# egor-achkasov/hermespy-rt

Hardware: AMD Instinct MI355X
Metric: resolved propagation paths/sec (higher is better)
Workload: dtype f32; 1 GPU; simple_street_canyon_with_cars.hrt, 1 TX + 4 RX, 4000000 rays/TX, 4 bounces, 3.5 GHz; parallelism=ray-sharded x1 (weak scaling), round-robin 4096-path granules, rays_total=4000000

## Files before the change

hermespy-rt_amd/csrc/host/problem.c:

```c
#include <math.h>
#include <pthread.h>
#include <stdarg.h>
#include <stdio.h>
#include <stdlib.h>
#include <string.h>
#include <time.h>
#include <unistd.h>

#include "hrt_internal.h"
#include "hrt_launch_plan.h"


static __thread char g_err[512];

const char *hrt_last_error(void) { return g_err; }
const char *hrt_version(void) { return "hermespy-rt_amd 0.1 (gfx950)"; }

int hrt_fail(int code, const char *fmt, ...)
{
    va_list ap;
    va_start(ap, fmt);
    vsnprintf(g_err, sizeof g_err, fmt, ap);
    va_end(ap);
    return code;
// ... 1267 lines not shown
{
    HRT_HIP(hrt_hip_set_device(device), "hipSetDevice");
    HRT_HIP(hrt_hip_free(ptr), "hipFree");
    return HRT_OK;
}
int hrt_device_upload(int device, void *dst, const void *src, uint64_t bytes)
{
    HRT_HIP(hrt_hip_set_device(device), "hipSetDevice");
    HRT_HIP(hrt_hip_h2d(dst, src, bytes), "hipMemcpy H2D");
    return HRT_OK;
}
int hrt_device_download(int device, void *dst, const void *src, uint64_t bytes)
{
    HRT_HIP(hrt_hip_set_device(device), "hipSetDevice");
    HRT_HIP(hrt_hip_d2h(dst, src, bytes), "hipMemcpy D2H");
    return HRT_OK;
}
int hrt_device_sync(int device, void *stream)
{
    HRT_HIP(hrt_hip_set_device(device), "hipSetDevice");
    HRT_HIP(hrt_hip_stream_sync(stream), "hipStreamSynchronize");
    return HRT_OK;
}
int hrt_device_mem_info(int device, uint64_t *free_bytes, uint64_t *total_bytes)
{
    HRT_HIP(hrt_hip_set_device(device), "hipSetDevice");
    HRT_HIP(hrt_hip_mem_info(free_bytes, total_bytes), "hipMemGetInfo");
    return HRT_OK;
}


int hrt_selftest_math(int device, int fn, const float *in, float *out, uint64_t n)
{
    if (!in || !out || fn < 0 || fn > 10) return hrt_fail(HRT_E_INVALID, "hrt_selftest_math: bad argument");
    void *d_in = NULL, *d_out = NULL;
    int rc = hrt_device_malloc(device, &d_in, n * 4);
    if (rc) return rc;
    if ((rc = hrt_device_malloc(device, &d_out, n * 4))) { hrt_device_free(device, d_in); return rc; }
    if (!(rc = hrt_device_upload(device, d_in, in, n * 4))) {
        int e = hrt_hip_selftest_math(fn, (const float *)d_in, (float *)d_out, n, NULL);
        if (e) rc = hrt_fail_hip(e, "hrt_selftest_math");
        else if (!(rc = hrt_device_sync(device, NULL))) rc = hrt_device_download(device, out, d_out, n * 4);
    }
    hrt_device_free(device, d_in);
    hrt_device_free(device, d_out);
    return rc;
}


static const void *cand_table(const hrt_problem *p, int mode)
{
    switch (mode) {
    case 0: return p->kpatch.mask;
    case 1: return p->kpatch.num_img ? p->kpatch.mask : NULL;
    case 2: return p->kpatch.txcell;
    case 3: return p->krxt.cell_mask;
    default: return NULL;
    }
}

int hrt_debug_candidates(const hrt_problem *p, int mode, uint64_t n, const float *in, uint32_t *out)
{
    if (!p || !in || !out || mode < 0 || mode > 3) return hrt_fail(HRT_E_INVALID, "hrt_debug_candidates: bad argument");
    if (n > (1ull << 26)) return hrt_fail(HRT_E_INVALID, "hrt_debug_candidates: more than 2^26 queries");
    if (!cand_table(p, mode)) return hrt_fail(HRT_E_INVALID, "hrt_debug_candidates: the problem has no table for mode %d", mode);
    if (n == 0) return HRT_OK;
    void *d_in = NULL, *d_out = NULL;
    int rc = hrt_device_malloc(p->device, &d_in, n * 32);
    if (rc) return rc;
    if ((rc = hrt_device_malloc(p->device, &d_out, n * 40))) { hrt_device_free(p->device, d_in); return rc; }
    if (!(rc = hrt_device_upload(p->device, d_in, in, n * 32))) {
        int e = hrt_hip_debug_candidates(p->d_tri, p->num_tri, p->d_tx_pos, p->num_rx, p->num_tx, &p->kpatch, &p->krxt, mode, n,
                                         (const float *)d_in, (uint32_t *)d_out, NULL);
// ... 41 lines not shown
```

hermespy-rt_amd/csrc/hrt_fused_body.inc:

```
    constexpr int AUX = CHAIN ? 16 : 0;
    const uint32_t tid = threadIdx.x, lane = tid & 63u, wave = tid >> 6;
    uint32_t *counts = reinterpret_cast<uint32_t *>(P.ws + P.off_counts);
    if (!CHAIN && FIRST && blockIdx.x >= gridDim.x - P.los_blocks) {
        los_pairs(P, blockIdx.x - (gridDim.x - P.los_blocks));
        return;
    }
    const uint32_t n_in = CHAIN ? n_in_c : (FIRST ? P.n0 : counts[b]);
    if (!CHAIN && !FIRST && (counts[P.num_bounces + 1] & kErrVoid)) return;
    const uint32_t n_grid = gridDim.x - (FIRST ? P.los_blocks : 0u);
    const uint32_t Ke = CHAIN ? Ke_c : ((K > 1 && n_in <= kShortList && (uint64_t)n_grid * HRT_BLOCK >= n_in) ? 1u : (uint32_t)K);
    const uint32_t MC = Ke * HRT_BLOCK;
    const uint32_t n_chunks = CHAIN ? n_chunks_c : (n_in + MC - 1u) / MC;
    const uint32_t chunk = CHAIN ? chunk_c : blockIdx.x;
    if (!CHAIN && chunk >= n_chunks) return;
    const bool do_trace = FIRST || (b < P.num_bounces);

    const uint32_t T = P.num_tri;
    const uint32_t cap4 = (uint32_t)P.cap * 4u;
    const float4 *g_tri = reinterpret_cast<const float4 *>(P.tri);
    const float2 *g_tg = reinterpret_cast<const float2 *>(P.acc.tg);
    const float4 *g_leaf = reinterpret_cast<const float4 *>(P.acc.leaf);
    const uint32_t n_leaf = P.acc.num_leaf;
    const FusedLds L = fused_lds<TRI_IN_LDS, (VARIANT == 9), FIRST>(lds, T, n_leaf, P.num_rx, wave);
#ifdef HRT_PHASE_STATS
// ... 142 lines not shown

    if constexpr (!FIRST) if (!P.records_done) {
        const uint32_t pb = b - 1;
#pragma unroll
        for (int k = 0; k < K; ++k) {
            const uint32_t i = chunk * MC + (uint32_t)k * HRT_BLOCK + tid;
            const uint32_t i4 = i * 4u;
            if (HRT_BALLOT(valid[k]) == 0ull) continue;
            const Ball ball = (VARIANT >= 2 && VARIANT != 6 && !masked) ? origin_ball(o[k], valid[k])
                                                                       : Ball{{0.f, 0.f, 0.f}, 0.f, false};
            F3 n = {0.f, 0.f, 1.f}, mvel = {0.f, 0.f, 0.f};
            float mat_s = 0.f, mat_alpha = 1.f, th = theta[k];
            if (valid[k]) {
                uint32_t ht = htri[k];
                if (ht >= T) {
                    atomicOr(&counts[P.num_bounces + 1], 4u);
                    ht = 0u;
                }
                const float4 q2 = tri[HRT_ROW * ht + 2];
                n = {q2.y, q2.z, q2.w};
                const uint32_t mesh = __float_as_uint(tri[HRT_ROW * ht + 4].w);
                const float4 mm = gather4(mesh_r, HRT_MESH_FLOATS * 4u, mesh, 0u);
                mvel = {mm.x, mm.y, mm.z};
                const float4 m3 = L.mat[4u * __float_as_uint(mm.w) + 3u];
                mat_s = m3.x;
                mat_alpha = m3.y;
            }
            for (uint32_t rx = 0; rx < P.num_rx; ++rx) {
                const float4 rp = L.rx[rx];
                const F3 apex = {rp.x, rp.y, rp.z};
                float d2rx;
                F3 w = shadow_dir(o[k], apex, d2rx);
                if (!valid[k]) w = {0.f, 0.f, 1.f};
                const Hit sh = masked ? closest_hit_masked(tri, P.acc.orig, P.rxt, rx, T, o[k], w, valid[k], lane, 2)
                                      : closest_hit<VARIANT>(tri, tg, leaf, P.acc, P.rxt, rx, P.acc.orig, T, o[k], w, valid[k],
                                                             lane, ball, true, apex, L.mask, L.wleaf, 2);
                bool unblocked = false;
                if (valid[k]) {
                    const Rsrc rec = rec_blk(P, pb, rx);
                    if (sh.tri != HRT_NO_HIT) {
                        const float4 s2 = tri[HRT_ROW * sh.tri + 2];
                        th = incidence_angle({s2.y, s2.z, s2.w}, w);
                    }
                    if (sh.tri != HRT_NO_HIT && sh.t <= 1.f) {
                        stf(rec, R_A0 * cap4, i4, 0.f);
                        stf(rec, R_A1 * cap4, i4, 0.f);
                        stf(rec, R_A2 * cap4, i4, 0.f);
                        stf(rec, R_A3 * cap4, i4, 0.f);
                        stf(rec, R_TAU * cap4, i4, 0.f);
                    } else {
                        unblocked = true;
                        const float th_s = acos_f_ool(dot3(w, n));
                        const float4 S = scatter_pattern(mat_s, mat_alpha, th_s, th, lds_addr(L.mat + kMatItems));
                        float o0 = a0[k] * S.x - a1[k] * S.y;
                        float o1 = a0[k] * S.y + a1[k] * S.x;
                        float o2 = a2[k] * S.z - a3[k] * S.w;
                        float o3 = a2[k] * S.w + a3[k] * S.z;
                        float f2 = P.fsl_mult * d2rx;
                        f2 *= f2;
                        if (f2 > 1.f) { o0 /= f2; o1 /= f2; o2 /= f2; o3 /= f2; }
                        stf(rec, R_A0 * cap4, i4, o0);
                        stf(rec, R_A1 * cap4, i4, o1);
                        stf(rec, R_A2 * cap4, i4, o2);
                        stf(rec, R_A3 * cap4, i4, o3);
                        stf(rec, R_TAU * cap4, i4, tau[k] + div_c(d2rx));
                        stf(rec, R_DX * cap4, i4, -w.x);
                        stf(rec, R_DY * cap4, i4, -w.y);
// ... 71 lines not shown
```

hermespy-rt_amd/csrc/hrt_kernels.hip:

```cpp
#include <hip/hip_runtime.h>
#include <string.h>

#include <stdint.h>
#include <stdio.h>
#include <stdlib.h>

#include "hrt_kparams.h"
#include "hrt_launch_dir.h"
#include "hrt_launch_plan.h"
#include "hrt_libm.h"

#pragma clang fp contract(off)

namespace {

constexpr float kEps = 1.1920928955078125e-07f;
constexpr float kOnePlusEps = 1.00000011920928955078125f;
constexpr float kPi = 3.14159265358979323846f;
constexpr float kC = 299792458.0f;
constexpr float kInvC = 1.0f / kC;
__device__ __forceinline__ float div_c(float a)
{
    const float q = a * kInvC;
    const float r = __builtin_fmaf(-q, kC, a);
// ... 21 lines not shown
template <typename TriPtr>
__device__ __forceinline__ Hit closest_hit_plain(TriPtr tri, const uint32_t *__restrict__ orig,
                                                 uint32_t num_tri, F3 o, F3 d)
{
    float best = 1e9f;
    uint32_t who = HRT_NO_HIT, who_o = 0u;
    for (uint32_t j = 0; j < num_tri; ++j) {
        const float4 q0 = tri[HRT_ROW * j], q1 = tri[HRT_ROW * j + 1], q2 = tri[HRT_ROW * j + 2];
        const F3 v1 = {q0.x, q0.y, q0.z};
        const F3 e1 = {q0.w, q1.x, q1.y};
        const F3 e2 = {q1.z, q1.w, q2.x};
        const F3 pv = cross3(d, e2);
        const float det = dot3(e1, pv);
        if (det > -kEps && det < kEps) continue;
        const F3 s = sub3(o, v1);
        const float u = dot3(s, pv) / det;
        if (u < -kEps || u > kOnePlusEps) continue;
        const F3 q = cross3(s, e1);
        const float v = dot3(d, q) / det;
        const float w = u + v;
        if (v < -kEps || w > kOnePlusEps) continue;
        const float dist = dot3(e2, q) / det;
        if (dist > kEps && (dist < best || (dist == best && orig[j] < who_o))) {
            best = dist; who = j; who_o = orig[j];
        }
    }
    return {who, best};
}

constexpr float kK1 = 1.1920928955078125e-07f * (1.f + 0x1p-18f);
constexpr float kK2 = 1.f + 0x1p-20f;
constexpr float kK3 = 1.f + 0x1p-19f;
constexpr float kK5 = 1.1920928955078125e-07f * (1.f - 0x1p-18f);

__device__ __forceinline__ uint32_t lane_prefix(unsigned long long mask)
{
    return __builtin_amdgcn_mbcnt_hi((uint32_t)(mask >> 32),
                                     __builtin_amdgcn_mbcnt_lo((uint32_t)mask, 0u));
}

__device__ __forceinline__ bool wave_all(bool p) { return __builtin_amdgcn_ballot_w64(!p) == 0ull; }

__device__ __forceinline__ float xor_sign(float x, uint32_t sign_bit)
{
    return __uint_as_float(__float_as_uint(x) ^ sign_bit);
}

template <typename TriPtr>
__device__ __forceinline__ Hit closest_hit_staged(TriPtr tri, const uint32_t *__restrict__ orig,
                                                  uint32_t num_tri, F3 o, F3 d)
{
    float best = 1e9f;
    uint32_t who = HRT_NO_HIT, who_o = 0u;
    for (uint32_t j = 0; j < num_tri; ++j) {
        const float4 q0 = tri[HRT_ROW * j], q1 = tri[HRT_ROW * j + 1], q2 = tri[HRT_ROW * j + 2];
        const F3 v1 = {q0.x, q0.y, q0.z};
        const F3 e1 = {q0.w, q1.x, q1.y};
        const F3 e2 = {q1.z, q1.w, q2.x};
        const F3 pv = cross3(d, e2);
        const float det = dot3(e1, pv);
        const F3 s = sub3(o, v1);
        const float nu = dot3(s, pv);
        const float a = fabsf(det);
        const uint32_t sg = __float_as_uint(det) & 0x80000000u;
        const float nu_s = xor_sign(nu, sg);
        const float k1a = kK1 * a, k2a = kK2 * a;
// ... 319 lines not shown
#define HRT_STAGED_BODY(J)                                                                      \
    {                                                                                           \
        const float4 q0 = tri[HRT_ROW * (J)], q1 = tri[HRT_ROW * (J) + 1], q2 = tri[HRT_ROW * (J) + 2];           \
        HRT_STAGED_TEST(J, q0, q1, q2)                                                          \
    }
#define HRT_STAGED_TEST(J, q0, q1, q2)                                                          \
    {                                                                                           \
        const F3 v1 = {q0.x, q0.y, q0.z};                                                       \
        const F3 e1 = {q0.w, q1.x, q1.y};                                                       \
        const F3 e2 = {q1.z, q1.w, q2.x};                                                       \
        const F3 pv = cross3(d, e2);                                                            \
        const float det = dot3(e1, pv);                                                         \
        const F3 s = sub3(o, v1);                                                               \
        const float nu = dot3(s, pv);                                                           \
        const float a = fabsf(det);                                                             \
        const uint32_t sg = __float_as_uint(det) & 0x80000000u;                                 \
        const float nu_s = xor_sign(nu, sg);                                                    \
        const float k1a = kK1 * a, k2a = kK2 * a;                                               \
        unsigned long long rm = inval | HRT_BALLOT(a < kEps) | HRT_BALLOT(nu_s < -k1a) |        \
                                HRT_BALLOT(nu_s > k2a);                                         \
        if (rm != ~0ull) {                                                                      \
            HRT_STAT(kind, 3, 1);                                                               \
            const F3 q = cross3(s, e1);                                                         \
            const float nv = dot3(d, q);                                                        \
            const float nv_s = xor_sign(nv, sg);                                                \
            rm |= HRT_BALLOT(nv_s < -k1a) | HRT_BALLOT((nu_s + nv_s) > kK3 * a);                \
            if (rm != ~0ull) {                                                                  \
                HRT_STAT(kind, 4, 1);                                                           \
                const float nt = dot3(e2, q);                                                   \
                const float nt_s = xor_sign(nt, sg);                                            \
                rm |= HRT_BALLOT(nt_s < kK5 * a) | HRT_BALLOT(nt_s > (best * a) * kK2);         \
                if (rm != ~0ull) {                                                              \
                    HRT_STAT(kind, 5, 1);                                                       \
                    const float u = nu / det;                                                   \
                    const float v = nv / det;                                                   \
                    const float w = u + v;                                                      \
                    const float dist = nt / det;                                                \
                    const bool rej = (rm >> lane) & 1ull;                                       \
                    const bool miss = (det > -kEps && det < kEps) | (u < -kEps) |               \
                                      (u > kOnePlusEps) | (v < -kEps) | (w > kOnePlusEps);      \
                    const uint32_t oj = orig[(J)];         \
                    const bool take = !rej & !miss & (dist > kEps) &                            \
                                      ((dist < best) | ((dist == best) & (oj < who_o)));        \
                    best = take ? dist : best;                                                  \
                    who = take ? (J) : who;                                                     \
                    who_o = take ? oj : who_o;                                                  \
                }                                                                               \
            }                                                                                   \
        }                                                                                       \
    }

constexpr uint32_t kMaskRounds = HRT_MASK_ROUNDS;
constexpr uint32_t kCandBuf = HRT_CAND_BUF;
__host__ __device__ constexpr uint32_t wave_scratch4(bool cand_buf) { return HRT_WAVE_SCRATCH4(cand_buf); }

__device__ __forceinline__ uint32_t rxt_cell(F3 a)
{
    const float ax = fabsf(a.x), ay = fabsf(a.y), az = fabsf(a.z);
    uint32_t m = 0u;
    float major = a.x, c1 = a.y, c2 = a.z;
    if (ay > ax && ay >= az) { m = 1u; major = a.y; c1 = a.z; c2 = a.x; }
    else if (az > ax && az > ay) { m = 2u; major = a.z; c1 = a.x; c2 = a.y; }
    const float inv = __builtin_amdgcn_rcpf(major);
    const float u = c1 * inv, v = c2 * inv;
    int iu = (int)((u * 0.5f + 0.5f) * (float)HRT_RXT_N), iv = (int)((v * 0.5f + 0.5f) * (float)HRT_RXT_N);
    iu = iu < 0 ? 0 : (iu > HRT_RXT_N - 1 ? HRT_RXT_N - 1 : iu);
    iv = iv < 0 ? 0 : (iv > HRT_RXT_N - 1 ? HRT_RXT_N - 1 : iv);
    const uint32_t f = m + (major < 0.f ? 3u : 0u);
    return (f * HRT_RXT_N + (uint32_t)iv) * HRT_RXT_N + (uint32_t)iu;
}

__device__ __forceinline__ bool rxt_inside(const hrt_krxt &X, F3 o)
{
    const F3 dc = sub3(o, {X.cx, X.cy, X.cz});
    return fast_sqrt(fdot3(dc, dc)) * 1.0001f <= X.region_r;
}
__device__ __forceinline__ unsigned long long rxt_cell_load(const hrt_krxt &X, uint32_t apex_k, F3 d)
{
    return X.cell_mask[(uint64_t)apex_k * HRT_RXT_BINS + rxt_cell(d)];
}
template <typename TriPtr>
__device__ __forceinline__ Hit closest_hit_masked(TriPtr tri, const uint32_t *__restrict__ orig, const hrt_krxt &X,
                                                  uint32_t apex_k, uint32_t num_tri, F3 o, F3 d, bool valid,
                                                  uint32_t lane, [[maybe_unused]] int kind)
{
    float best = 1e9f;
    uint32_t who = HRT_NO_HIT, who_o = 0u;
    const unsigned long long inval = HRT_BALLOT(!valid);
    if (inval == ~0ull) return {who, best};
    unsigned long long mine = 0ull;
    if (valid) {
        mine = rxt_inside(X, o) ? rxt_cell_load(X, apex_k, d)
                                : (num_tri >= 64u ? ~0ull : ((1ull << num_tri) - 1ull));
    }
    unsigned long long m = wave_or64(mine);
    HRT_STAT(kind, 0, 1);
    HRT_STAT(kind, 1, 1);
    HRT_STAT(kind, 2, __popcll(m));
    while (m) {
        const uint32_t j = (uint32_t)__builtin_ctzll(m);
        m &= m - 1ull;
        HRT_STAGED_BODY(j)
    }
    return {who, best};
}

using Rsrc = __amdgpu_buffer_rsrc_t;
__device__ __forceinline__ Rsrc make_rsrc(const uint8_t *base)
{
    return __builtin_amdgcn_make_buffer_rsrc(const_cast<uint8_t *>(base), 0, 0xffffffff, 0x00020000);
}

__device__ __forceinline__ void wave_or256(uint32_t (&w)[8])
{
    uint32_t c[4];
#pragma unroll
    for (int k = 0; k < 4; ++k) {
        const auto r = __builtin_amdgcn_permlane32_swap(w[k], w[k + 4], false, false);
        c[k] = (uint32_t)r[0] | (uint32_t)r[1];
    }
    uint32_t e[2];
#pragma unroll
    for (int k = 0; k < 2; ++k) {
        const auto r = __builtin_amdgcn_permlane16_swap(c[k], c[k + 2], false, false);
        e[k] = (uint32_t)r[0] | (uint32_t)r[1];
    }
#define HRT_OR2(CTRL) "v_or_b32_dpp %0, %0, %0 " CTRL "\n" "v_or_b32_dpp %1, %1, %1 " CTRL "\n" "s_nop 0\n"
    asm volatile(
        "s_nop 4\n"
        HRT_OR2("row_shr:1 row_mask:0xf bank_mask:0xf")
        HRT_OR2("row_shr:2 row_mask:0xf bank_mask:0xf")
// ... 34 lines not shown
        const float fu = fdot3(sv, {p0.x, p0.y, p0.z}), fv = fdot3(sv, {p1.x, p1.y, p1.z});
        const float hh = fdot3(sv, {q2.y, q2.z, q2.w});
        const uint32_t bits = __float_as_uint(p1.w), nu = bits & 0xffffu, nv = bits >> 16;
        R.served = (nu != 0u) & (fabsf(hh) <= X.hmax) & (fu >= -HRT_PATCH_ACCEPT) & (fv >= -HRT_PATCH_ACCEPT) &
                   (fu <= (float)nu + HRT_PATCH_ACCEPT) & (fv <= (float)nv + HRT_PATCH_ACCEPT);
        if (image) {
            const F3 im = image_of(apex, q0, q2);
            const F3 wv = sub3(o, im);
            const F3 cx = fcross3(wv, d);
            R.served &= (fdot3(cx, cx) <= 0.98f * X.ro_img * X.ro_img) && (fdot3(wv, d) > 0.f);
        }
        const uint32_t iu = min((uint32_t)max((int)floorf(fu), 0), nu - 1u);
        const uint32_t iv = min((uint32_t)max((int)floorf(fv), 0), nv - 1u);
        R.off = (__float_as_uint(p0.w) + iv * nu + iu) * (HRT_PATCH_WORDS * 8u);
    }
    return R;
}

__device__ __forceinline__ void patch_load(const hrt_kpatch &X, const PatchRef R, uint32_t apex_k, bool valid, uint32_t (&w)[8])
{
#pragma unroll
    for (int k = 0; k < 8; ++k) w[k] = 0u;
    if (valid && R.served) {
        const Rsrc mr = make_rsrc(reinterpret_cast<const uint8_t *>(X.mask));
        const uint32_t off = R.off + apex_k * X.num_patch * (HRT_PATCH_WORDS * 8u);
        const auto a = __builtin_amdgcn_raw_buffer_load_b128(mr, (int)off, 0, 0);
        const auto b = __builtin_amdgcn_raw_buffer_load_b128(mr, (int)(off + 16u), 0, 0);
        w[0] = (uint32_t)a[0]; w[1] = (uint32_t)a[1]; w[2] = (uint32_t)a[2]; w[3] = (uint32_t)a[3];
        w[4] = (uint32_t)b[0]; w[5] = (uint32_t)b[1]; w[6] = (uint32_t)b[2]; w[7] = (uint32_t)b[3];
    }
}
__device__ __forceinline__ bool patch_whole(const PatchRef R, bool valid) { return HRT_BALLOT(valid && !R.served) != 0ull; }

template <typename TriPtr, typename OrigPtr>
__device__ __forceinline__ Hit closest_hit_words(TriPtr tri, OrigPtr orig, uint32_t (&w)[8], const bool whole, uint32_t num_tri,
                                                 F3 o, F3 d, bool valid, uint32_t lane, [[maybe_unused]] int kind)
{
    float best = 1e9f;
    uint32_t who = HRT_NO_HIT, who_o = 0u;
    const unsigned long long inval = HRT_BALLOT(!valid);
    if (inval == ~0ull) return {who, best};
    wave_or256(w);
    if (whole) {
#pragma unroll
        for (int k = 0; k < 8; ++k)
            w[k] |= num_tri >= 32u * (uint32_t)(k + 1) ? ~0u : (num_tri > 32u * (uint32_t)k ? (1u << (num_tri - 32u * (uint32_t)k)) - 1u : 0u);
    }
    HRT_STAT(kind, 0, 1);
    HRT_STAT(kind, 1, 1);
#pragma unroll
    for (uint32_t r = 0; r < HRT_PATCH_WORDS; ++r) {
        unsigned long long m = ((unsigned long long)w[2u * r + 1u] << 32) | (unsigned long long)w[2u * r];
        HRT_STAT(kind, 2, __popcll(m));
        while (m) {
            const uint32_t j = r * 64u + (uint32_t)__builtin_ctzll(m);
            m &= m - 1ull;
            HRT_STAGED_BODY(j)
        }
    }
    return {who, best};
}

template <typename TriPtr, typename OrigPtr>
__device__ __forceinline__ Hit closest_hit_patch(TriPtr tri, OrigPtr orig, const hrt_kpatch &X,
                                                 const PatchRef R, uint32_t apex_k, uint32_t num_tri, F3 o, F3 d,
                                                 bool valid, uint32_t lane, [[maybe_unused]] int kind)
{
    uint32_t w[8];
    patch_load(X, R, apex_k, valid, w);
    HRT_STAT(kind, 6, (valid && R.served) ? 1 : 0);
    return closest_hit_words(tri, orig, w, patch_whole(R, valid), num_tri, o, d, valid, lane, kind);
}

__device__ __forceinline__ void txcell_load(const hrt_kpatch &X, uint32_t tx, F3 d, uint32_t (&w)[8])
{
    const Rsrc mr = make_rsrc(reinterpret_cast<const uint8_t *>(X.txcell));
    const uint32_t off = (tx * HRT_RXT_BINS + rxt_cell(d)) * (HRT_PATCH_WORDS * 8u);
    const auto a = __builtin_amdgcn_raw_buffer_load_b128(mr, (int)off, 0, 0);
    const auto b = __builtin_amdgcn_raw_buffer_load_b128(mr, (int)(off + 16u), 0, 0);
    w[0] = (uint32_t)a[0]; w[1] = (uint32_t)a[1]; w[2] = (uint32_t)a[2]; w[3] = (uint32_t)a[3];
    w[4] = (uint32_t)b[0]; w[5] = (uint32_t)b[1]; w[6] = (uint32_t)b[2]; w[7] = (uint32_t)b[3];
}

template <typename TriPtr, typename OrigPtr>
__device__ __forceinline__ Hit closest_hit_txcell(TriPtr tri, OrigPtr orig, const hrt_kpatch &X, uint32_t tx, uint32_t num_tri,
                                                  F3 o, F3 d, bool valid, uint32_t lane)
{
    uint32_t w[8];
#pragma unroll
    for (int k = 0; k < 8; ++k) w[k] = 0u;
    if (valid) txcell_load(X, tx, d, w);
    return closest_hit_words(tri, orig, w, false, num_tri, o, d, valid, lane, 0);
}

template <bool MULTI, typename TriPtr>
__device__ __forceinline__ Hit closest_hit_packet(TriPtr tri, const uint32_t *__restrict__ orig,
                                                  const hrt_krxt &X, uint32_t rxk,
                                                  uint32_t num_tri, F3 o, F3 d,
                                                  bool valid, uint32_t lane, const Ball &B,
                                                  const bool shadow, F3 apex,
                                                  unsigned long long *wmask, int kind)
{
    float best = 1e9f;
    uint32_t who = HRT_NO_HIT, who_o = 0u;
// ... 1764 lines not shown
        PatchRef ref = {false, 0u};
        if (valid) {
            float4 pd0, pd1;
            patch_fetch(P.patch, T, htri, true, pd0, pd1);
            float4 mm = make_float4(0.f, 0.f, 0.f, 0.f);
            if (htri < T) mm = gather4(mesh_r, HRT_MESH_FLOATS * 4u, __float_as_uint(tri[HRT_ROW * htri + 4].w), 0u);
            ref = patch_locate(tri, P.patch, T, htri, o, false, o, o, pd0, pd1);
            if (htri < T) {
                const float4 q2 = tri[HRT_ROW * htri + 2];
                n = {q2.y, q2.z, q2.w};
                mvel = {mm.x, mm.y, mm.z};
                const float4 m3 = l_mat[4u * __float_as_uint(mm.w) + 3u];
                mat_s = m3.x;
                mat_alpha = m3.y;
            }
        }
#if HRT_RECORDS_PREFETCH
        uint32_t wnext[8];
        patch_load(P.patch, ref, 0u, valid, wnext);
        const bool whole = patch_whole(ref, valid);
#pragma unroll
        for (int q = 0; q < 8; ++q) asm volatile("" : "+v"(wnext[q]));
#endif
        for (uint32_t rx = 0; rx < P.num_rx; ++rx) {
            const float4 rp = l_rx[rx];
            float d2rx;
            F3 w = shadow_dir(o, {rp.x, rp.y, rp.z}, d2rx);
            if (!valid) w = {0.f, 0.f, 1.f};
#if HRT_RECORDS_PREFETCH
            uint32_t wcur[8];
#pragma unroll
            for (int q = 0; q < 8; ++q) wcur[q] = wnext[q];
            if (rx + 1u < P.num_rx) patch_load(P.patch, ref, rx + 1u, valid, wnext);
            const Hit h = closest_hit_words(tri, l_orig, wcur, whole, T, o, w, valid, lane, 2);
#pragma unroll
            for (int q = 0; q < 8; ++q) asm volatile("" : "+v"(wnext[q]));
#else
            const Hit h = closest_hit_patch(tri, l_orig, P.patch, ref, rx, T, o, w, valid, lane, 2);
#endif
            bool unblocked = false;
            if (valid) {
                if (h.tri != HRT_NO_HIT) {
                    const float4 q2 = tri[HRT_ROW * h.tri + 2];
                    theta = incidence_angle({q2.y, q2.z, q2.w}, w);
                }
                if (h.tri != HRT_NO_HIT && h.t <= 1.f) {
                    stf(rec_blk(P, pb, rx), R_A0 * cap4, i4, 0.f);
                    stf(rec_blk(P, pb, rx), R_A1 * cap4, i4, 0.f);
                    stf(rec_blk(P, pb, rx), R_A2 * cap4, i4, 0.f);
                    stf(rec_blk(P, pb, rx), R_A3 * cap4, i4, 0.f);
                    stf(rec_blk(P, pb, rx), R_TAU * cap4, i4, 0.f);
                } else {
                    unblocked = true;
                    const float th_s = acos_f_ool(dot3(w, n));
                    const float4 S = scatter_pattern(mat_s, mat_alpha, th_s, theta, lds_addr(l_mat + kMatItems));
                    float o0 = a0 * S.x - a1 * S.y;
                    float o1 = a0 * S.y + a1 * S.x;
                    float o2 = a2 * S.z - a3 * S.w;
                    float o3 = a2 * S.w + a3 * S.z;
                    float f2 = P.fsl_mult * d2rx;
                    f2 *= f2;
                    if (f2 > 1.f) { o0 /= f2; o1 /= f2; o2 /= f2; o3 /= f2; }
                    stf(rec_blk(P, pb, rx), R_A0 * cap4, i4, o0);
                    stf(rec_blk(P, pb, rx), R_A1 * cap4, i4, o1);
                    stf(rec_blk(P, pb, rx), R_A2 * cap4, i4, o2);
                    stf(rec_blk(P, pb, rx), R_A3 * cap4, i4, o3);
                    stf(rec_blk(P, pb, rx), R_TAU * cap4, i4, tau + div_c(d2rx));
                    stf(rec_blk(P, pb, rx), R_DX * cap4, i4, -w.x);
                    stf(rec_blk(P, pb, rx), R_DY * cap4, i4, -w.y);
                    stf(rec_blk(P, pb, rx), R_DZ * cap4, i4, -w.z);
                    stf(rec_blk(P, pb, rx), R_DFS * cap4, i4, dot3(sub3(w, d), mvel) * P.dop_mult);
// ... 973 lines not shown
    }
}

__global__ void hrt_selftest_math_kernel(int fn, const float *in, float *out, uint64_t n)
{
    const uint64_t i = (uint64_t)blockIdx.x * blockDim.x + threadIdx.x;
    __shared__ uint64_t l_exp[HRT_EXP2_TAB_BYTES / 8u];
    if (threadIdx.x < HRT_EXP2_TAB_BYTES / 8u) l_exp[threadIdx.x] = hrt_exp2_tab(threadIdx.x);
    __syncthreads();
    if (fn >= 8) {
        selftest_items(fn, in, out, n, i, lds_addr(l_exp));
        return;
    }
    if (i >= n) return;
    const float x = in[i];
    float y;
    switch (fn) {
    case 0: y = hrt_sinf(x); break;
    case 1: y = hrt_cosf(x); break;
    case 2: y = hrt_expf_lds(x, lds_addr(l_exp)); break;
    case 3: y = hrt_acosf(x); break;
    case 5: { float c_; hrt_sincosf(x, &y, &c_); break; }
    case 6: { float s_; hrt_sincosf(x, &s_, &y); break; }
    case 7: y = hrt_cosf_nb(x); break;
    default: {
        float th = (float)acos((double)x);
        if (th > kPi * 0.5f) th = kPi - th;
        y = th;
    }
    }
    out[i] = y;
}

__global__ __launch_bounds__(256) void hrt_debug_candidates_kernel(const float *tri_f, uint32_t num_tri, const float *tx_pos,
                                                                   uint32_t num_rx, uint32_t num_tx, const hrt_kpatch X,
                                                                   const hrt_krxt R, int mode, uint64_t n, const float *in,
                                                                   uint32_t *out)
{
    const uint64_t i = (uint64_t)blockIdx.x * 256u + threadIdx.x;
    if (i >= n) return;
    const float4 *tri = reinterpret_cast<const float4 *>(tri_f);
    const float *q = in + 8u * i;
    const F3 o = {q[0], q[1], q[2]}, d = {q[3], q[4], q[5]};
    const uint32_t row = __float_as_uint(q[6]), apex = __float_as_uint(q[7]);
    uint32_t w[8];
#pragma unroll
    for (int k = 0; k < 8; ++k) w[k] = 0u;
    uint32_t served = 0u, pidx = 0u;
    if (mode <= 1) {
        const bool image = mode == 1;
        const bool ok = apex < (image ? X.num_img : num_rx);
        float4 p0, p1;
        patch_fetch(X, num_tri, row, true, p0, p1);
        F3 ap = o;
        if (image && ok) ap = {tx_pos[3u * apex], tx_pos[3u * apex + 1u], tx_pos[3u * apex + 2u]};
        PatchRef ref = patch_locate(tri, X, num_tri, row, o, image, ap, image ? d : o, p0, p1);
        ref.served = ref.served && ok;
        patch_load(X, ref, image ? num_rx + apex : apex, true, w);
        served = ref.served ? 1u : 0u;
        pidx = ref.served ? ref.off / (HRT_PATCH_WORDS * 8u) : 0u;
    } else if (mode == 2) {
        if (apex < num_tx) {
            txcell_load(X, apex, d, w);
            served = 1u;
        }
    } else {
// ... 480 lines not shown
}
int hrt_hip_d2d_async(void *dst, const void *src, uint64_t bytes, void *stream)
{
    return (int)hipMemcpyAsync(dst, src, bytes, hipMemcpyDeviceToDevice, (hipStream_t)stream);
}

int hrt_hip_launch_fs0(const float *d_dirs, uint64_t n, const float *tx_vel3, float mult, float *d_out, void *stream)
{
    if (n == 0) return 0;
    hipLaunchKernelGGL(hrt_fs0_kernel, dim3((uint32_t)((n + 255) / 256)), dim3(256), 0, (hipStream_t)stream,
                       d_dirs, n, tx_vel3[0], tx_vel3[1], tx_vel3[2], mult, d_out);
    return (int)hipGetLastError();
}

int hrt_hip_launch_order(const uint32_t *d_seg_start, const uint32_t *d_seg_band, uint32_t num_seg,
                         uint64_t num_paths, uint32_t rank, uint32_t count, uint32_t chunk,
                         uint32_t *d_order, void *stream)
{
    if (num_seg == 0) return 0;
    {
        const hipError_t e = hipFuncSetAttribute(reinterpret_cast<const void *>(&hrt_launch_order_kernel),
                                                 hipFuncAttributeMaxDynamicSharedMemorySize,
                                                 (int)(HRT_ORDER_SEG * 4u));
        if (e != hipSuccess) return (int)e;
    }
    hipLaunchKernelGGL(hrt_launch_order_kernel, dim3(num_seg), dim3(1024), HRT_ORDER_SEG * 4u,
                       (hipStream_t)stream, d_seg_start, d_seg_band, num_paths, rank, count, chunk, d_order);
    return (int)hipGetLastError();
}

int hrt_hip_selftest_math(int fn, const float *d_in, float *d_out, uint64_t n, void *stream)
{
    if (n == 0) return 0;
    hipLaunchKernelGGL(hrt_selftest_math_kernel, dim3((uint32_t)((n + 255) / 256)), dim3(256), 0,
                       (hipStream_t)stream, fn, d_in, d_out, n);
    return (int)hipGetLastError();
}

int hrt_hip_debug_candidates(const float *d_tri, uint32_t num_tri, const float *d_tx_pos, uint32_t num_rx, uint32_t num_tx,
                             const hrt_kpatch *patch, const hrt_krxt *rxt, int mode, uint64_t n, const float *d_in,
                             uint32_t *d_out, void *stream)
{
    if (n == 0) return 0;
    hipLaunchKernelGGL(hrt_debug_candidates_kernel, dim3((uint32_t)((n + 255) / 256)), dim3(256), 0, (hipStream_t)stream,
                       d_tri, num_tri, d_tx_pos, num_rx, num_tx, *patch, *rxt, mode, n, d_in, d_out);
    return (int)hipGetLastError();
}

int hrt_hip_read_stats(unsigned long long *out, int reset)
{
#ifdef HRT_PHASE_STATS
    if (const char *pf = getenv("HRT_PHASE_FILE")) {
        static unsigned long long host_phase[65536][8];
        if (hipMemcpyFromSymbol(host_phase, HIP_SYMBOL(g_phase), sizeof host_phase) == hipSuccess) {
            if (FILE *f = fopen(pf, "wb")) { fwrite(host_phase, 1, sizeof host_phase, f); fclose(f); }
        }
    }
#endif
#ifdef HRT_UNIT_CLOCKS
    if (const char *uf = getenv("HRT_UNIT_FILE")) {
        static unsigned long long host_unit[1u << 21][2];
        unsigned int n = 0;
        if (hipMemcpyFromSymbol(&n, HIP_SYMBOL(g_unit_n), sizeof n) == hipSuccess &&
            hipMemcpyFromSymbol(host_unit, HIP_SYMBOL(g_unit), sizeof host_unit) == hipSuccess) {
            if (n > (1u << 21)) n = 1u << 21;
            if (FILE *f = fopen(uf, "wb")) { fwrite(host_unit, 16, n, f); fclose(f); }
// ... 60 lines not shown
```

profiles/accel_stats.py:

```python
#!/usr/bin/env python3
import ctypes
import json
import os
import sys
import tempfile

sys.path.insert(0, os.path.dirname(os.path.dirname(os.path.abspath(__file__))))
import torch
from hermespy_rt_amd import lib
from hermespy_rt_amd.device import Tracer
from tests import scenes_gen as G

p = os.path.join(tempfile.mkdtemp(), "room.hrt")
if sys.argv[1] in ("c1", "c2", "c3", "c4", "c5"):
    from hermespy_rt_amd.workloads import WORKLOADS
    w = WORKLOADS[sys.argv[1]]
    T = -1
    tr = Tracer(w["scene_path"], w["rx_pos"], w["tx_pos"], w["rx_vel"], w["tx_vel"], w["f_ghz"], w["num_paths"], w["num_bounces"])
elif os.environ.get("HRT_SCALING_SCENE", "room") == "city":
    nb = int(sys.argv[1])
    rays = int(sys.argv[2]) if len(sys.argv) > 2 else 200000
    T, _ = G.city(p, nb)
    tr = Tracer(p, [[60.0, 0.0, 1.5], [0.0, -90.0, 1.5], [-150.0, 30.0, 1.5]], [[0.0, 0.0, 25.0]], [[0, 0, 0]] * 3,
                [[0, 0, 0]], 3.5, rays, 2)
else:
    nb = int(sys.argv[1])
    rays = int(sys.argv[2]) if len(sys.argv) > 2 else 200000
    T = G.room_with_clutter(p, nb, seed=7, tilt=True, scale=max(1.0, (nb / 500.0) ** (1.0 / 3.0)))
    tr = Tracer(p, [[5, 3, 1.5], [-8, -4, 2.0], [12, 9, 8.0]], [[-10, 5, 6.0]], [[0, 0, 0]] * 3, [[0, 0, 0]], 3.5, rays, 2)
arr = (ctypes.c_uint64 * 48)()
lib.load().hrt_debug_kernel_stats(0, arr, 1)
tr.trace()
torch.cuda.synchronize()
lib.load().hrt_debug_kernel_stats(0, arr, 0)
cols = ["wave_traces", "usable_full", "candidates", "stage2", "stage3", "exact", "subpackets", "cull_rounds",
        "sphere_rounds", "plane_rounds", "plane_leaves", "plane_leaves_flagged", "flagged", "max_clk", "sum_clk"]
cols = cols[:13] + ["max_clk", "sum_clk", "clk15"]
for k, name in enumerate(("primary0", "primary", "shadow")):
    row = {c: int(arr[k * 16 + j]) for j, c in enumerate(cols)}
    wt = max(1, row["wave_traces"])
    row["per_trace"] = {c: round(row[c] / wt, 2) for c in cols[1:]}
    print(json.dumps(dict(T=T, kind=name, variant=os.environ.get("HRT_TUNE", "default"), **row)))
```

Baseline: 30.46 billion paths/s.

## Skip divisions in triangle tests via certified division-free barycentric and distance checks

Adds certification bands so the exact Möller-Trumbore stage skips the u/v divisions when a wave-wide ballot shows every candidate is certainly inside the triangle. For shadow rays, adds a pair-valued (numerator, |det|) best-hit tracker that compares by cross-multiplication, so the per-hit distance division is skipped unless a comparison falls in an uncertain band. Shadow paths through the masked and patch walkers now use this variant. A selftest walk kernel is added to check equivalence. The aim is to cut divide cost in the hot intersection loop, at the price of extra ballots and some code complexity.

```diff
diff --git a/hermespy-rt_amd/csrc/host/problem.c b/hermespy-rt_amd/csrc/host/problem.c
--- a/hermespy-rt_amd/csrc/host/problem.c
+++ b/hermespy-rt_amd/csrc/host/problem.c
@@ -1323,13 +1323,14 @@
 
 int hrt_selftest_math(int device, int fn, const float *in, float *out, uint64_t n)
 {
-    if (!in || !out || fn < 0 || fn > 10) return hrt_fail(HRT_E_INVALID, "hrt_selftest_math: bad argument");
+    if (!in || !out || fn < 0 || fn > 11) return hrt_fail(HRT_E_INVALID, "hrt_selftest_math: bad argument");
     void *d_in = NULL, *d_out = NULL;
     int rc = hrt_device_malloc(device, &d_in, n * 4);
     if (rc) return rc;
     if ((rc = hrt_device_malloc(device, &d_out, n * 4))) { hrt_device_free(device, d_in); return rc; }
     if (!(rc = hrt_device_upload(device, d_in, in, n * 4))) {
-        int e = hrt_hip_selftest_math(fn, (const float *)d_in, (float *)d_out, n, NULL);
+        int e = hrt_hip_memset_async(d_out, 0, n * 4, NULL);
+        if (!e) e = hrt_hip_selftest_math(fn, (const float *)d_in, (float *)d_out, n, NULL);
         if (e) rc = hrt_fail_hip(e, "hrt_selftest_math");
         else if (!(rc = hrt_device_sync(device, NULL))) rc = hrt_device_download(device, out, d_out, n * 4);
     }
diff --git a/hermespy-rt_amd/csrc/hrt_fused_body.inc b/hermespy-rt_amd/csrc/hrt_fused_body.inc
--- a/hermespy-rt_amd/csrc/hrt_fused_body.inc
+++ b/hermespy-rt_amd/csrc/hrt_fused_body.inc
@@ -198,7 +198,7 @@
                 float d2rx;
                 F3 w = shadow_dir(o[k], apex, d2rx);
                 if (!valid[k]) w = {0.f, 0.f, 1.f};
-                const Hit sh = masked ? closest_hit_masked(tri, P.acc.orig, P.rxt, rx, T, o[k], w, valid[k], lane, 2)
+                const Hit sh = masked ? closest_hit_masked<true>(tri, P.acc.orig, P.rxt, rx, T, o[k], w, valid[k], lane, 2)
                                       : closest_hit<VARIANT>(tri, tg, leaf, P.acc, P.rxt, rx, P.acc.orig, T, o[k], w, valid[k],
                                                              lane, ball, true, apex, L.mask, L.wleaf, 2);
                 bool unblocked = false;
diff --git a/hermespy-rt_amd/csrc/hrt_kernels.hip b/hermespy-rt_amd/csrc/hrt_kernels.hip
--- a/hermespy-rt_amd/csrc/hrt_kernels.hip
+++ b/hermespy-rt_amd/csrc/hrt_kernels.hip
@@ -77,6 +77,8 @@
 constexpr float kK2 = 1.f + 0x1p-20f;
 constexpr float kK3 = 1.f + 0x1p-19f;
 constexpr float kK5 = 1.1920928955078125e-07f * (1.f - 0x1p-18f);
+constexpr float kCertW = 1.f - 0x1p-20f;
+constexpr float kCertMaxDet = 0x1p126f;
 
 __device__ __forceinline__ uint32_t lane_prefix(unsigned long long mask)
 {
@@ -462,13 +464,22 @@
                 rm |= HRT_BALLOT(nt_s < kK5 * a) | HRT_BALLOT(nt_s > (best * a) * kK2);         \
                 if (rm != ~0ull) {                                                              \
                     HRT_STAT(kind, 5, 1);                                                       \
-                    const float u = nu / det;                                                   \
-                    const float v = nv / det;                                                   \
-                    const float w = u + v;                                                      \
+                    const unsigned long long unc =                                              \
+                        ~rm & (HRT_BALLOT(!(nu_s >= 0.f)) | HRT_BALLOT(!(nv_s >= 0.f)) |        \
+                               HRT_BALLOT(!((nu_s + nv_s) <= kCertW * a)) |                     \
+                               HRT_BALLOT(!(a <= kCertMaxDet)));                                \
+                    bool miss = false;                                                          \
+                    if (unc != 0ull) {     \
+                        const float u = nu / det;                                               \
+                        const float v = nv / det;                                               \
+                        const float w = u + v;                                                  \
+                        miss = (det > -kEps && det < kEps) | (u < -kEps) |                      \
+                               (u > kOnePlusEps) | (v < -kEps) | (w > kOnePlusEps);             \
+                    } else {                                                                    \
+                        HRT_STAT(kind, 15, 1);                                                  \
+                    }                                                                           \
                     const float dist = nt / det;                                                \
                     const bool rej = (rm >> lane) & 1ull;                                       \
-                    const bool miss = (det > -kEps && det < kEps) | (u < -kEps) |               \
-                                      (u > kOnePlusEps) | (v < -kEps) | (w > kOnePlusEps);      \
                     const uint32_t oj = orig[(J)];         \
                     const bool take = !rej & !miss & (dist > kEps) &                            \
                                       ((dist < best) | ((dist == best) & (oj < who_o)));        \
@@ -479,6 +490,80 @@
             }                                                                                   \
         }                                                                                       \
     }
+
+constexpr float kK5H = 1.1920928955078125e-07f * (1.f + 0x1p-18f);
+constexpr float kPairMax = 0x1p120f;
+#define HRT_STAGED_BODY_S(J)                                                                    \
+    {                                                                                           \
+        const float4 q0 = tri[HRT_ROW * (J)], q1 = tri[HRT_ROW * (J) + 1], q2 = tri[HRT_ROW * (J) + 2];           \
+        const F3 v1 = {q0.x, q0.y, q0.z};                                                       \
+        const F3 e1 = {q0.w, q1.x, q1.y};                                                       \
+        const F3 e2 = {q1.z, q1.w, q2.x};                                                       \
+        const F3 pv = cross3(d, e2);                                                            \
+        const float det = dot3(e1, pv);                                                         \
+        const F3 s = sub3(o, v1);                                                               \
+        const float nu = dot3(s, pv);                                                           \
+        const float a = fabsf(det);                                                             \
+        const uint32_t sg = __float_as_uint(det) & 0x80000000u;                                 \
+        const float nu_s = xor_sign(nu, sg);                                                    \
+        const float k1a = kK1 * a, k2a = kK2 * a;                                               \
+        unsigned long long rm = inval | HRT_BALLOT(a < kEps) | HRT_BALLOT(nu_s < -k1a) |        \
+                                HRT_BALLOT(nu_s > k2a);                                         \
+        if (rm != ~0ull) {                                                                      \
+            HRT_STAT(kind, 3, 1);                                                               \
+            const F3 q = cross3(s, e1);                                                         \
+            const float nv = dot3(d, q);                                                        \
+            const float nv_s = xor_sign(nv, sg);                                                \
+            rm |= HRT_BALLOT(nv_s < -k1a) | HRT_BALLOT((nu_s + nv_s) > kK3 * a);                \
+            if (rm != ~0ull) {                                                                  \
+                HRT_STAT(kind, 4, 1);                                                           \
+                const float nt = dot3(e2, q);                                                   \
+                const float nt_s = xor_sign(nt, sg);                                            \
+                const float pn = nt_s * a_b, po = nt_b * a;                                     \
+                rm |= HRT_BALLOT(nt_s < kK5 * a) | HRT_BALLOT(pn > po * kK2);                   \
+                if (rm != ~0ull) {                                                              \
+                    HRT_STAT(kind, 5, 1);                                                       \
+                    const unsigned long long unc =                                              \
+                        ~rm & (HRT_BALLOT(!(nu_s >= 0.f)) | HRT_BALLOT(!(nv_s >= 0.f)) |        \
+                               HRT_BALLOT(!((nu_s + nv_s) <= kCertW * a)) |                     \
+                               HRT_BALLOT(!(a <= kCertMaxDet)));                                \
+                    bool miss = false;                                                          \
+                    if (unc != 0ull) {     \
+                        const float u = nu / det;                                               \
+                        const float v = nv / det;                                               \
+                        const float w = u + v;                                                  \
+                        miss = (det > -kEps && det < kEps) | (u < -kEps) |                      \
+                               (u > kOnePlusEps) | (v < -kEps) | (w > kOnePlusEps);             \
+                    } else {                                                                    \
+                        HRT_STAT(kind, 15, 1);                                                  \
+                    }                                                                           \
+                    const unsigned long long band =                                             \
+                        ~rm & (HRT_BALLOT(!(nt_s > kK5H * a)) | HRT_BALLOT(!(pn < po * kCertW)) | \
+                               HRT_BALLOT(!(po <= kPairMax)));                                  \
+                    const bool rej = (rm >> lane) & 1ull;                                       \
+                    const uint32_t oj = orig[(J)];         \
+                    bool take = !rej & !miss;                                                   \
+                    if (band != 0ull) {        \
+                        const float dist = nt / det;                                            \
+                        const float bq = nt_b / a_b;                                            \
+                        take = take & (dist > kEps) &                                           \
+                               ((dist < bq) | ((dist == bq) & (oj < who_o)));                   \
+                    }                                                                           \
+                    nt_b = take ? nt_s : nt_b;                                                  \
+                    a_b = take ? a : a_b;                                                       \
+                    who = take ? (J) : who;                                                     \
+                    who_o = take ? oj : who_o;                                                  \
+                }                                                                               \
+            }                                                                                   \
+        }                                                                                       \
+    }
+__device__ __forceinline__ Hit shadow_result(uint32_t who, float nt_b, float a_b)
+{
+    const bool yes = nt_b <= a_b * kCertW, no = nt_b > a_b * kK2;
+    bool within = yes;
+    if (HRT_BALLOT(!yes & !no) != 0ull) within = yes | (!no & (nt_b / a_b <= 1.f));
+    return {who, within ? 0.f : 2.f};
+}
 
 constexpr uint32_t kMaskRounds = HRT_MASK_ROUNDS;
 constexpr uint32_t kCandBuf = HRT_CAND_BUF;
@@ -509,7 +594,7 @@
 {
     return X.cell_mask[(uint64_t)apex_k * HRT_RXT_BINS + rxt_cell(d)];
 }
-template <typename TriPtr>
+template <bool PAIR = false, typename TriPtr>
 __device__ __forceinline__ Hit closest_hit_masked(TriPtr tri, const uint32_t *__restrict__ orig, const hrt_krxt &X,
                                                   uint32_t apex_k, uint32_t num_tri, F3 o, F3 d, bool valid,
                                                   uint32_t lane, [[maybe_unused]] int kind)
@@ -527,6 +612,15 @@
     HRT_STAT(kind, 0, 1);
     HRT_STAT(kind, 1, 1);
     HRT_STAT(kind, 2, __popcll(m));
+    if constexpr (PAIR) {
+        float nt_b = 1e9f, a_b = 1.f;
+        while (m) {
+            const uint32_t j = (uint32_t)__builtin_ctzll(m);
+            m &= m - 1ull;
+            HRT_STAGED_BODY_S(j)
+        }
+        return shadow_result(who, nt_b, a_b);
+    }
     while (m) {
         const uint32_t j = (uint32_t)__builtin_ctzll(m);
         m &= m - 1ull;
@@ -627,7 +721,7 @@
 }
 __device__ __forceinline__ bool patch_whole(const PatchRef R, bool valid) { return HRT_BALLOT(valid && !R.served) != 0ull; }
 
-template <typename TriPtr, typename OrigPtr>
+template <bool PAIR = false, typename TriPtr, typename OrigPtr>
 __device__ __forceinline__ Hit closest_hit_words(TriPtr tri, OrigPtr orig, uint32_t (&w)[8], const bool whole, uint32_t num_tri,
                                                  F3 o, F3 d, bool valid, uint32_t lane, [[maybe_unused]] int kind)
 {
@@ -643,6 +737,7 @@
     }
     HRT_STAT(kind, 0, 1);
     HRT_STAT(kind, 1, 1);
+    [[maybe_unused]] float nt_b = 1e9f, a_b = 1.f;
 #pragma unroll
     for (uint32_t r = 0; r < HRT_PATCH_WORDS; ++r) {
         unsigned long long m = ((unsigned long long)w[2u * r + 1u] << 32) | (unsigned long long)w[2u * r];
@@ -650,13 +745,14 @@
         while (m) {
             const uint32_t j = r * 64u + (uint32_t)__builtin_ctzll(m);
             m &= m - 1ull;
-            HRT_STAGED_BODY(j)
-        }
-    }
+            if constexpr (PAIR) HRT_STAGED_BODY_S(j) else HRT_STAGED_BODY(j)
+        }
+    }
+    if constexpr (PAIR) return shadow_result(who, nt_b, a_b);
     return {who, best};
 }
 
-template <typename TriPtr, typename OrigPtr>
+template <bool PAIR = false, typename TriPtr, typename OrigPtr>
 __device__ __forceinline__ Hit closest_hit_patch(TriPtr tri, OrigPtr orig, const hrt_kpatch &X,
                                                  const PatchRef R, uint32_t apex_k, uint32_t num_tri, F3 o, F3 d,
                                                  bool valid, uint32_t lane, [[maybe_unused]] int kind)
@@ -664,7 +760,7 @@
     uint32_t w[8];
     patch_load(X, R, apex_k, valid, w);
     HRT_STAT(kind, 6, (valid && R.served) ? 1 : 0);
-    return closest_hit_words(tri, orig, w, patch_whole(R, valid), num_tri, o, d, valid, lane, kind);
+    return closest_hit_words<PAIR>(tri, orig, w, patch_whole(R, valid), num_tri, o, d, valid, lane, kind);
 }
 
 __device__ __forceinline__ void txcell_load(const hrt_kpatch &X, uint32_t tx, F3 d, uint32_t (&w)[8])
@@ -2495,11 +2591,11 @@
 #pragma unroll
             for (int q = 0; q < 8; ++q) wcur[q] = wnext[q];
             if (rx + 1u < P.num_rx) patch_load(P.patch, ref, rx + 1u, valid, wnext);
-            const Hit h = closest_hit_words(tri, l_orig, wcur, whole, T, o, w, valid, lane, 2);
+            const Hit h = closest_hit_words<true>(tri, l_orig, wcur, whole, T, o, w, valid, lane, 2);
 #pragma unroll
             for (int q = 0; q < 8; ++q) asm volatile("" : "+v"(wnext[q]));
 #else
-            const Hit h = closest_hit_patch(tri, l_orig, P.patch, ref, rx, T, o, w, valid, lane, 2);
+            const Hit h = closest_hit_patch<true>(tri, l_orig, P.patch, ref, rx, T, o, w, valid, lane, 2);
 #endif
             bool unblocked = false;
             if (valid) {
@@ -3539,6 +3635,40 @@
     out[i] = y;
 }
 
+struct InlineOrig {
+    const float *rows;
+    __device__ __forceinline__ uint32_t operator[](uint32_t j) const { return __float_as_uint(rows[HRT_TRI_FLOATS * j + HRT_TRI_FLOATS - 1u]); }
+};
+constexpr uint64_t kWalkItem = 8u + 8u * HRT_TRI_FLOATS;
+static_assert(kWalkItem == 168u && HRT_TRI_FLOATS % 4u == 0u, "selftest walk item: 16-byte aligned rows");
+__global__ __launch_bounds__(256) void hrt_selftest_walk_kernel(const float *in, float *out, uint64_t n)
+{
+    const uint64_t i = (uint64_t)blockIdx.x * 256u + threadIdx.x;
+    const uint64_t items = n / kWalkItem;
+    if ((i & ~(uint64_t)63) >= items) return;
+    const bool live = i < items;
+    const uint32_t lane = threadIdx.x & 63u;
+    const float *it = in + kWalkItem * (live ? i : 0u);
+    const F3 o = {it[0], it[1], it[2]}, d = {it[3], it[4], it[5]};
+    const uint32_t kind = __float_as_uint(it[6]);
+    const uint32_t T = min(__float_as_uint(it[7]), 8u);
+    const float4 *tri = reinterpret_cast<const float4 *>(it + 8);
+    const InlineOrig orig = {it + 8};
+    Hit h = {HRT_NO_HIT, 1e9f};
+#pragma unroll
+    for (int k = 0; k < 3; k += 2) {
+        const bool mine = live && kind == (uint32_t)k;
+        uint32_t w[8] = {mine ? (1u << T) - 1u : 0u, 0u, 0u, 0u, 0u, 0u, 0u, 0u};
+        const Hit g = k == 2 ? closest_hit_words<true>(tri, orig, w, false, 8u, o, d, mine, lane, 2)
+                             : closest_hit_words(tri, orig, w, false, 8u, o, d, mine, lane, 0);
+        if (mine) h = g;
+    }
+    if (live) {
+        out[kWalkItem * i] = __uint_as_float(h.tri);
+        out[kWalkItem * i + 1u] = kind == 2u ? __uint_as_float(h.t <= 1.f ? 1u : 0u) : h.t;
+    }
+}
+
 __global__ __launch_bounds__(256) void hrt_debug_candidates_kernel(const float *tri_f, uint32_t num_tri, const float *tx_pos,
                                                                    uint32_t num_rx, uint32_t num_tx, const hrt_kpatch X,
                                                                    const hrt_krxt R, int mode, uint64_t n, const float *in,
@@ -4085,6 +4215,13 @@
 int hrt_hip_selftest_math(int fn, const float *d_in, float *d_out, uint64_t n, void *stream)
 {
     if (n == 0) return 0;
+    if (fn == 11) {
+        const uint64_t items = n / kWalkItem;
+        if (items == 0) return 0;
+        hipLaunchKernelGGL(hrt_selftest_walk_kernel, dim3((uint32_t)((items + 255) / 256)), dim3(256), 0,
+                           (hipStream_t)stream, d_in, d_out, n);
+        return (int)hipGetLastError();
+    }
     hipLaunchKernelGGL(hrt_selftest_math_kernel, dim3((uint32_t)((n + 255) / 256)), dim3(256), 0,
                        (hipStream_t)stream, fn, d_in, d_out, n);
     return (int)hipGetLastError();
diff --git a/profiles/accel_stats.py b/profiles/accel_stats.py
--- a/profiles/accel_stats.py
+++ b/profiles/accel_stats.py
@@ -30,12 +30,17 @@
     tr = Tracer(p, [[5, 3, 1.5], [-8, -4, 2.0], [12, 9, 8.0]], [[-10, 5, 6.0]], [[0, 0, 0]] * 3, [[0, 0, 0]], 3.5, rays, 2)
 arr = (ctypes.c_uint64 * 48)()
 lib.load().hrt_debug_kernel_stats(0, arr, 1)
-tr.trace()
-torch.cuda.synchronize()
+for attempt in range(3):
+    tr.trace()
+    torch.cuda.synchronize()
+    if not (tr.error_word() & 0x300):
+        break
+    print("void step (error word %#x): counting again" % tr.error_word(), file=sys.stderr)
+    lib.load().hrt_debug_kernel_stats(0, arr, 1)
 lib.load().hrt_debug_kernel_stats(0, arr, 0)
 cols = ["wave_traces", "usable_full", "candidates", "stage2", "stage3", "exact", "subpackets", "cull_rounds",
         "sphere_rounds", "plane_rounds", "plane_leaves", "plane_leaves_flagged", "flagged", "max_clk", "sum_clk"]
-cols = cols[:13] + ["max_clk", "sum_clk", "clk15"]
+cols = cols[:13] + ["max_clk", "sum_clk", "exact_certain"]
 for k, name in enumerate(("primary0", "primary", "shadow")):
     row = {c: int(arr[k * 16 + j]) for j, c in enumerate(cols)}
     wt = max(1, row["wave_traces"])
```

Measured after the change: 30.91 billion paths/s (median of 6 runs). 1.5% higher.
